# customink/lambdipy

Hardware: NVIDIA H100
Metric: ELF-strip GB/s (build-tree .so bytes) (higher is better)
Workload: dtype u8

## Files before the change

### lambdipy_b200/csrc/api.cu

```cuda
#include "lb2_common.cuh"
#include "../../include/lambdipy_b200.h"

#include <algorithm>
#include <atomic>
#include <chrono>
#include <cctype>
#include <cerrno>
#include <cstdio>
#include <cstdlib>
#include <condition_variable>
#include <cstring>
#include <mutex>
#include <string>
#include <thread>
#include <vector>

#include <climits>
#include <dirent.h>
#include <regex.h>
#include <fcntl.h>
#include <spawn.h>
#include <sys/stat.h>
#include <sys/syscall.h>
#include <sys/wait.h>
// ... 1 lines not shown

extern char **environ;

using namespace lb2;

static thread_local std::string g_create_error;

struct Workspace {
  uint64_t *d_in_off = nullptr, *d_in_size = nullptr, *d_out_size = nullptr, *d_out_off = nullptr;
  int32_t *d_status = nullptr;
  uint8_t *d_scratch = nullptr;
  Tile *d_tiles = nullptr;
  BatchCounters *d_ctr = nullptr;
  UpRange *d_ranges = nullptr, *h_ranges = nullptr;
  BigExt *d_big = nullptr;
  uint32_t cap_big = 0;
  uint32_t cap_ranges = 0;
  uint64_t *h_stage = nullptr;
  uint8_t *h_res = nullptr;
  BatchCounters *h_ctr = nullptr;
  cudaEvent_t done = nullptr;
  uint32_t cap_files = 0;
  uint64_t cap_tiles = 0;
  cudaEvent_t ev[3] = {nullptr, nullptr, nullptr};
  uint32_t n_files = 0;
  cudaStream_t stream = nullptr;
  bool in_flight = false;
};

struct TreeEngine;
struct lb2_ctx {
  int device = 0;
  int numa_node = -1;
  int sm_count = 0;
  cudaStream_t stream = nullptr;
  Workspace ws;
  Workspace ws2;
  int async_head = 0, async_count = 0;
  std::string err;
  int compact_ctas_per_sm = 4;
  int use_tma = 1;
  struct Slot {
    Workspace ws;
    cudaStream_t stream = nullptr;
    uint8_t *d_in = nullptr, *d_out = nullptr;
    uint64_t cap_in = 0, cap_out = 0;
    cudaEvent_t ev_h2d[2] = {nullptr, nullptr}, ev_d2h[2] = {nullptr, nullptr}, ev_planned = nullptr;
  } slot[3];
  TreeEngine *tree = nullptr;
};
struct TreeEngine;
static void tree_engine_free(TreeEngine *e);

#define CK(call)                                                                                   \
  do {                                                                                             \
    cudaError_t e_ = (call);                                                                       \
    if (e_ != cudaSuccess) {                                                                       \
      ctx->err = std::string(#call) + ": " + cudaGetErrorString(e_);                               \
      return LB2_E_CUDA;                                                                           \
    }                                                                                              \
  } while (0)

static int gpu_numa_node(int device) {
  char bus[64] = {0};
  if (cudaDeviceGetPCIBusId(bus, sizeof bus, device) != cudaSuccess) { cudaGetLastError(); return -1; }
  for (char *c = bus; *c; c++) *c = (char)tolower(*c);
  std::string path = std::string("/sys/bus/pci/devices/") + bus + "/numa_node";
  FILE *f = fopen(path.c_str(), "r");
  if (!f) return -1;
  int node = -1;
  if (fscanf(f, "%d", &node) != 1) node = -1;
// ... 23 lines not shown
  for (uint32_t i = t; i <= n; i += stride) h_off[i] = out_off[i];
  for (uint32_t i = t; i < n; i += stride) { h_size[i] = out_size[i]; h_status[i] = status[i]; }
  if (ranges) {
    const uint32_t nr = ctr->n_ranges < range_cap ? ctr->n_ranges : range_cap;
    for (uint32_t i = t; i < nr; i += stride) h_ranges[i] = ranges[i];
  }
}

static double now_s() {
  return std::chrono::duration<double>(std::chrono::steady_clock::now().time_since_epoch()).count();
}

static void ws_free(Workspace &w) {
  cudaFree(w.d_in_off); cudaFree(w.d_in_size); cudaFree(w.d_out_size); cudaFree(w.d_out_off); cudaFree(w.d_status);
  cudaFree(w.d_scratch); cudaFree(w.d_tiles); cudaFree(w.d_ctr);
  if (w.h_stage) cudaFreeHost(w.h_stage);
  if (w.h_res) cudaFreeHost(w.h_res);
  if (w.h_ctr) cudaFreeHost(w.h_ctr);
  cudaFree(w.d_ranges);
  cudaFree(w.d_big);
  if (w.h_ranges) cudaFreeHost(w.h_ranges);
  for (auto &e : w.ev) if (e) cudaEventDestroy(e);
  if (w.done) cudaEventDestroy(w.done);
  w = Workspace();
}

static int ws_reserve(lb2_ctx *ctx, Workspace &w, uint32_t n_files, uint64_t n_tiles) {
  if (!w.d_ctr) {
    CK(cudaMalloc(&w.d_ctr, sizeof(BatchCounters)));
    CK(cudaHostAlloc(&w.h_ctr, sizeof(BatchCounters) + 64, cudaHostAllocMapped));
    for (auto &e : w.ev) CK(cudaEventCreate(&e));
    CK(cudaEventCreateWithFlags(&w.done, cudaEventDisableTiming));
  }
  if (n_files > w.cap_files) {
    uint32_t cap = std::max<uint32_t>(n_files, 256u);
    cap = std::max<uint32_t>(cap, w.cap_files + w.cap_files / 2);
    cudaFree(w.d_in_off); cudaFree(w.d_in_size); cudaFree(w.d_out_size); cudaFree(w.d_out_off); cudaFree(w.d_status); cudaFree(w.d_scratch);
    if (w.h_stage) cudaFreeHost(w.h_stage);
    if (w.h_res) cudaFreeHost(w.h_res);
    w.h_stage = nullptr; w.h_res = nullptr;
    w.d_in_off = w.d_in_size = w.d_out_size = w.d_out_off = nullptr; w.d_status = nullptr; w.d_scratch = nullptr;
    w.cap_files = 0;
    CK(cudaMalloc(&w.d_in_off, (cap + 1) * sizeof(uint64_t)));
    CK(cudaMalloc(&w.d_in_size, (cap + 1) * sizeof(uint64_t)));
    CK(cudaMalloc(&w.d_out_size, (cap + 1) * sizeof(uint64_t)));
    CK(cudaMalloc(&w.d_out_off, (cap + 1) * sizeof(uint64_t)));
    CK(cudaMalloc(&w.d_status, (cap + 1) * sizeof(int32_t)));
    CK(cudaMalloc(&w.d_scratch, (uint64_t)cap * SCR_STRIDE));
    CK(cudaHostAlloc(&w.h_stage, (2ull * cap + 2) * sizeof(uint64_t), cudaHostAllocMapped));
    CK(cudaHostAlloc(&w.h_res, (2ull * cap + 2) * sizeof(uint64_t) + (cap + 1ull) * sizeof(int32_t), cudaHostAllocMapped));
    w.cap_files = cap;
  }
  if (n_tiles > w.cap_tiles) {
    uint64_t cap = std::max<uint64_t>(n_tiles, w.cap_tiles + w.cap_tiles / 2);
    cudaFree(w.d_tiles);
    w.d_tiles = nullptr;
    w.cap_tiles = 0;
    CK(cudaMalloc(&w.d_tiles, cap * sizeof(Tile)));
    w.cap_tiles = cap;
  }
  return LB2_OK;
}

static uint64_t tile_bound(const uint64_t *sizes, uint32_t n) {
  uint64_t t = 65536;
  for (uint32_t i = 0; i < n; i++) t += sizes[i] / TILE_BYTES + 2 * MAX_EXT + 16;
  return t;
}

static int enqueue_batch(lb2_ctx *ctx, Workspace &w, const uint8_t *d_in, const uint64_t *h_off, const uint64_t *h_sizes,
                         uint32_t n, uint8_t *d_out, uint64_t out_cap, uint32_t flags, cudaStream_t s, bool compact,
                         bool export_ranges = false, bool via_mapping = false) {
  for (uint32_t i = 0; i < n; i++)
    if (h_off[i] & 15) { ctx->err = "input offsets must be multiples of 16"; return LB2_E_ARG; }
  std::vector<uint64_t> tmp;
  if (w.in_flight) { ctx->err = "previous batch on this workspace not collected"; return LB2_E_STATE; }
  uint64_t *st_off = nullptr, *st_size = nullptr;
  {
    tmp.resize(n);
    for (uint32_t i = 0; i < n; i++) tmp[i] = h_sizes ? h_sizes[i] : (h_off[i + 1] - h_off[i]);
  }
  int rc = ws_reserve(ctx, w, n, tile_bound(tmp.data(), n));
  if (rc) return rc;
  st_off = w.h_stage;
  st_size = w.h_stage + (w.cap_files + 1);
  memcpy(st_off, h_off, (size_t)n * sizeof(uint64_t));
  memcpy(st_size, tmp.data(), (size_t)n * sizeof(uint64_t));
  const uint64_t *k_in_off = w.d_in_off, *k_in_size = w.d_in_size;
  if (via_mapping) {
    void *alias = nullptr;
    CK(cudaHostGetDevicePointer(&alias, w.h_stage, 0));
    k_in_off = static_cast<const uint64_t *>(alias);
    k_in_size = k_in_off + (w.cap_files + 1);
    lb2_zero_ctr_kernel<<<1, 64, 0, s>>>(w.d_ctr);
  } else {
    CK(cudaMemcpyAsync(w.d_in_off, st_off, (size_t)n * sizeof(uint64_t), cudaMemcpyHostToDevice, s));
    CK(cudaMemcpyAsync(w.d_in_size, st_size, (size_t)n * sizeof(uint64_t), cudaMemcpyHostToDevice, s));
    CK(cudaMemsetAsync(w.d_ctr, 0, sizeof(BatchCounters), s));
  }
  CK(cudaEventRecord(w.ev[0], s));
  if (export_ranges && w.cap_ranges < 8u * n + 4096u) {
    cudaFree(w.d_ranges);
    if (w.h_ranges) cudaFreeHost(w.h_ranges);
    w.d_ranges = nullptr; w.h_ranges = nullptr; w.cap_ranges = 0;
    const uint32_t cap = 8u * std::max<uint32_t>(n, w.cap_files) + 4096u;
    CK(cudaMalloc(&w.d_ranges, (size_t)cap * sizeof(UpRange)));
    CK(cudaHostAlloc(&w.h_ranges, (size_t)cap * sizeof(UpRange), cudaHostAllocMapped));
    w.cap_ranges = cap;
  }
  PlanArgs pa;
  pa.in = d_in; pa.in_off = k_in_off; pa.in_size = k_in_size; pa.n_files = n; pa.flags = flags;
  pa.scratch = w.d_scratch; pa.out_size = w.d_out_size; pa.status = w.d_status;
  pa.tiles = w.d_tiles; pa.tile_cap = w.cap_tiles; pa.ctr = w.d_ctr;
  pa.up_ranges = export_ranges ? w.d_ranges : nullptr; pa.up_cap = export_ranges ? w.cap_ranges : 0;
  if (w.cap_big < 8u * n + 4096u) {
    cudaFree(w.d_big);
    w.d_big = nullptr; w.cap_big = 0;
    const uint32_t cap = 8u * std::max<uint32_t>(n, w.cap_files) + 4096u;
    CK(cudaMalloc(&w.d_big, (size_t)cap * sizeof(BigExt)));
    w.cap_big = cap;
  }
  pa.big = w.d_big; pa.big_cap = w.cap_big;
  launch_plan(pa, s);
  launch_scan(w.d_out_size, w.d_out_off, n, compact ? out_cap : ~0ull, w.d_ctr, w.d_big, w.cap_big, w.d_tiles, ctx->sm_count * 2, s);
  CK(cudaEventRecord(w.ev[1], s));
  if (compact) {
    CompactArgs ca;
    ca.tiles = w.d_tiles; ca.ctr = w.d_ctr; ca.out_off = w.d_out_off; ca.out = d_out;
    ca.rebase_lo = ca.rebase_len = ca.rebase_delta = 0;
    if (ctx->use_tma) launch_compact_tma(ca, ctx->sm_count, s);
    else launch_compact(ca, ctx->sm_count * ctx->compact_ctas_per_sm, s);
  }
  CK(cudaEventRecord(w.ev[2], s));
  {
    uint64_t *r_off = reinterpret_cast<uint64_t *>(w.h_res), *r_size = r_off + (w.cap_files + 1);
    int32_t *r_status = reinterpret_cast<int32_t *>(r_size + (w.cap_files + 1));
    if (via_mapping) {
      void *a_ctr = nullptr, *a_res = nullptr, *a_rng = nullptr;
      CK(cudaHostGetDevicePointer(&a_ctr, w.h_ctr, 0));
      CK(cudaHostGetDevicePointer(&a_res, w.h_res, 0));
      if (export_ranges) CK(cudaHostGetDevicePointer(&a_rng, w.h_ranges, 0));
      uint64_t *m_off = static_cast<uint64_t *>(a_res), *m_size = m_off + (w.cap_files + 1);
      int32_t *m_status = reinterpret_cast<int32_t *>(m_size + (w.cap_files + 1));
      lb2_publish_kernel<<<std::max(1u, std::min(32u, (n + 255u) / 256u)), 256, 0, s>>>(
          w.d_ctr, w.d_out_off, w.d_out_size, w.d_status, export_ranges ? w.d_ranges : nullptr, n, w.cap_ranges,
          static_cast<BatchCounters *>(a_ctr), m_off, m_size, m_status, static_cast<UpRange *>(a_rng));
    } else {
      CK(cudaMemcpyAsync(w.h_ctr, w.d_ctr, sizeof(BatchCounters), cudaMemcpyDeviceToHost, s));
      if (export_ranges) CK(cudaMemcpyAsync(w.h_ranges, w.d_ranges, (size_t)std::min<uint32_t>(w.cap_ranges, 8u * n + 4096u) * sizeof(UpRange), cudaMemcpyDeviceToHost, s));
      CK(cudaMemcpyAsync(r_off, w.d_out_off, (size_t)(n + 1) * sizeof(uint64_t), cudaMemcpyDeviceToHost, s));
      if (n) {
        CK(cudaMemcpyAsync(r_size, w.d_out_size, (size_t)n * sizeof(uint64_t), cudaMemcpyDeviceToHost, s));
        CK(cudaMemcpyAsync(r_status, w.d_status, (size_t)n * sizeof(int32_t), cudaMemcpyDeviceToHost, s));
      }
    }
    CK(cudaEventRecord(w.done, s));
  }
  CK(cudaGetLastError());
  w.n_files = n;
  w.stream = s;
  w.in_flight = true;
  return LB2_OK;
}

static int collect_batch(lb2_ctx *ctx, Workspace &w, uint64_t *h_out_off, uint64_t *h_out_sizes, int32_t *h_status,
                         lb2_stats *stats) {
  if (!w.in_flight) { ctx->err = "no batch in flight"; return LB2_E_STATE; }
  const uint32_t n = w.n_files;
  CK(cudaEventSynchronize(w.done));
  w.in_flight = false;
  const uint64_t *r_off = reinterpret_cast<const uint64_t *>(w.h_res), *r_size = r_off + (w.cap_files + 1);
  const int32_t *r_status = reinterpret_cast<const int32_t *>(r_size + (w.cap_files + 1));
  if (h_out_off) memcpy(h_out_off, r_off, (size_t)(n + 1) * sizeof(uint64_t));
  if (h_out_sizes && n) memcpy(h_out_sizes, r_size, (size_t)n * sizeof(uint64_t));
  if (h_status && n) memcpy(h_status, r_status, (size_t)n * sizeof(int32_t));
  if (stats) {
    const BatchCounters &c = *w.h_ctr;
    memset(stats, 0, sizeof(*stats));
    stats->n_files = n; stats->n_ok = c.n_ok; stats->n_unsupported = c.n_unsupported; stats->overflow = c.overflow;
    stats->in_bytes = c.in_bytes; stats->out_bytes = c.out_bytes; stats->copy_bytes = c.copy_bytes;
    stats->header_bytes = c.header_bytes; stats->n_tiles = c.n_tiles; stats->out_bytes_needed = r_off[n];
    cudaEventElapsedTime(&stats->plan_ms, w.ev[0], w.ev[1]);
    cudaEventElapsedTime(&stats->compact_ms, w.ev[1], w.ev[2]);
  }
  if (w.h_ctr->overflow) { ctx->err = "output arena (or tile buffer) too small for this batch"; return LB2_E_CAPACITY; }
  return LB2_OK;
}

extern "C" {

const char *lb2_version(void) { return "lambdipy_b200 0.1 (sm_90a; GNU strip 2.42 semantics)"; }

int lb2_ctx_create(int device, lb2_ctx **out) {
  if (!out) return LB2_E_ARG;
  *out = nullptr;
  int count = 0;
  cudaError_t e = cudaGetDeviceCount(&count);
  if (e != cudaSuccess || count == 0) {
    g_create_error = std::string("no CUDA device: ") + (e != cudaSuccess ? cudaGetErrorString(e) : "device count is 0");
    return LB2_E_NODEVICE;
  }
  if (device < 0 || device >= count) { g_create_error = "device index out of range"; return LB2_E_ARG; }
  lb2_ctx *ctx = new lb2_ctx();
  ctx->device = device;
  if ((e = cudaSetDevice(device)) != cudaSuccess || (e = cudaStreamCreateWithFlags(&ctx->stream, cudaStreamNonBlocking)) != cudaSuccess) {
    g_create_error = std::string("cuda init: ") + cudaGetErrorString(e);
// ... 8 lines not shown
    g_create_error = "this library is built for sm_90a (H100) only; device is sm_" + std::to_string(prop.major) + std::to_string(prop.minor);
    cudaStreamDestroy(ctx->stream);
    delete ctx;
    return LB2_E_NODEVICE;
  }
  if (const char *v = getenv("LB2_COMPACT_CTAS_PER_SM")) ctx->compact_ctas_per_sm = std::max(1, atoi(v));
  if (const char *v = getenv("LB2_COMPACT_TMA")) ctx->use_tma = atoi(v);
  *out = ctx;
  return LB2_OK;
}

void lb2_ctx_destroy(lb2_ctx *ctx) {
  if (!ctx) return;
  cudaSetDevice(ctx->device);
  cudaDeviceSynchronize();
  ws_free(ctx->ws);
  ws_free(ctx->ws2);
  for (auto &sl : ctx->slot) {
    ws_free(sl.ws);
    cudaFree(sl.d_in); cudaFree(sl.d_out);
    if (sl.stream) cudaStreamDestroy(sl.stream);
    for (auto &e : sl.ev_h2d) if (e) cudaEventDestroy(e);
    for (auto &e : sl.ev_d2h) if (e) cudaEventDestroy(e);
    if (sl.ev_planned) cudaEventDestroy(sl.ev_planned);
  }
  tree_engine_free(ctx->tree);
  if (ctx->stream) cudaStreamDestroy(ctx->stream);
  delete ctx;
}

const char *lb2_last_error(const lb2_ctx *ctx) { return ctx ? ctx->err.c_str() : g_create_error.c_str(); }
int lb2_sm_count(const lb2_ctx *ctx) { return ctx ? ctx->sm_count : 0; }

void *lb2_dev_alloc(lb2_ctx *ctx, uint64_t bytes) {
  void *p = nullptr;
  cudaError_t e = cudaMalloc(&p, bytes ? bytes : 256);
  if (e != cudaSuccess) { if (ctx) ctx->err = std::string("cudaMalloc: ") + cudaGetErrorString(e); return nullptr; }
  return p;
}
void lb2_dev_free(lb2_ctx *, void *p) { if (p) cudaFree(p); }
void *lb2_pinned_alloc(lb2_ctx *ctx, uint64_t bytes) {
  void *p = nullptr;
  NumaPreferred near_gpu(ctx ? ctx->numa_node : -1);
  cudaError_t e = cudaHostAlloc(&p, bytes ? bytes : 256, cudaHostAllocMapped | cudaHostAllocPortable);
  if (e != cudaSuccess) { if (ctx) ctx->err = std::string("cudaHostAlloc: ") + cudaGetErrorString(e); return nullptr; }
  return p;
}
void lb2_pinned_free(lb2_ctx *, void *p) { if (p) cudaFreeHost(p); }
int lb2_memcpy_h2d(lb2_ctx *ctx, void *d, const void *h, uint64_t n) { CK(cudaMemcpy(d, h, n, cudaMemcpyHostToDevice)); return LB2_OK; }
int lb2_memcpy_d2h(lb2_ctx *ctx, void *h, const void *d, uint64_t n) { CK(cudaMemcpy(h, d, n, cudaMemcpyDeviceToHost)); return LB2_OK; }
int lb2_memset_d(lb2_ctx *ctx, void *d, int v, uint64_t n) { CK(cudaMemset(d, v, n)); return LB2_OK; }

int lb2_strip_device_async(lb2_ctx *ctx, const void *d_in, const uint64_t *h_in_off, const uint64_t *h_in_sizes,
                           uint32_t n_files, void *d_out, uint64_t out_capacity, uint32_t flags, void *stream) {
  if (!ctx || !d_in || !h_in_off || !d_out) { if (ctx) ctx->err = "NULL argument"; return LB2_E_ARG; }
  CK(cudaSetDevice(ctx->device));
  if (ctx->async_count >= 2) { ctx->err = "two batches already in flight: collect one with lb2_batch_results first"; return LB2_E_STATE; }
  cudaStream_t s = stream ? static_cast<cudaStream_t>(stream) : ctx->stream;
  Workspace &w = ((ctx->async_head + ctx->async_count) & 1) ? ctx->ws2 : ctx->ws;
  int rc = enqueue_batch(ctx, w, static_cast<const uint8_t *>(d_in), h_in_off, h_in_sizes, n_files,
                         static_cast<uint8_t *>(d_out), out_capacity, flags, s, true);
  if (rc == LB2_OK) ctx->async_count++;
  return rc;
}

int lb2_batch_results(lb2_ctx *ctx, uint64_t *h_out_off, uint64_t *h_out_sizes, int32_t *h_status, lb2_stats *stats) {
  if (!ctx) return LB2_E_ARG;
  if (ctx->async_count == 0) { ctx->err = "no batch in flight"; return LB2_E_STATE; }
  Workspace &w = (ctx->async_head & 1) ? ctx->ws2 : ctx->ws;
  ctx->async_head ^= 1;
  ctx->async_count--;
  return collect_batch(ctx, w, h_out_off, h_out_sizes, h_status, stats);
}

int lb2_plan_device(lb2_ctx *ctx, const void *d_in, const uint64_t *h_in_off, const uint64_t *h_in_sizes, uint32_t n_files,
                    uint32_t flags, uint64_t *h_out_sizes, int32_t *h_status, lb2_stats *stats) {
  if (!ctx || !d_in || !h_in_off) { if (ctx) ctx->err = "NULL argument"; return LB2_E_ARG; }
  CK(cudaSetDevice(ctx->device));
  if (ctx->async_count) { ctx->err = "batches of lb2_strip_device_async still in flight"; return LB2_E_STATE; }
  int rc = enqueue_batch(ctx, ctx->ws, static_cast<const uint8_t *>(d_in), h_in_off, h_in_sizes, n_files, nullptr, 0, flags,
                         ctx->stream, false);
  if (rc) return rc;
  return collect_batch(ctx, ctx->ws, nullptr, h_out_sizes, h_status, stats);
}
// ... 51 lines not shown
  for (size_t k = 0; k < chunks.size() && rc == LB2_OK; k++) {
    if (k >= 2) rc = collect(k - 2);
    if (rc == LB2_OK) rc = enqueue(k);
  }
  for (size_t k = chunks.size() >= 2 ? chunks.size() - 2 : 0; k < chunks.size(); k++) {
    Workspace &w = (k & 1) ? ctx->ws2 : ctx->ws;
    if (!w.in_flight) continue;
    int r = collect(k);
    if (rc == LB2_OK) rc = r;
  }
  if (total_out) *total_out = total;
  return rc;
}

static uint64_t env_u64(const char *name, uint64_t dflt) {
  const char *v = getenv(name);
  return v ? strtoull(v, nullptr, 10) : dflt;
}

static int strip_host_dma(lb2_ctx *ctx, const uint8_t *h_in, const uint8_t *d_in_alias, const uint64_t *h_in_off, const uint64_t *h_in_sizes,
                          uint32_t n_files, uint8_t *h_out, uint64_t out_capacity, uint64_t *h_out_off, uint64_t *h_out_sizes,
                          int32_t *h_status, uint32_t flags, lb2_stats *stats);

int lb2_strip_host(lb2_ctx *ctx, const void *h_in_v, const uint64_t *h_in_off, const uint64_t *h_in_sizes, uint32_t n_files,
                   void *h_out_v, uint64_t out_capacity, uint64_t *h_out_off, uint64_t *h_out_sizes, int32_t *h_status,
                   uint32_t flags, lb2_stats *stats) {
  if (!ctx || !h_in_v || !h_in_off || !h_out_v || !h_out_off || !h_out_sizes || !h_status) { if (ctx) ctx->err = "NULL argument"; return LB2_E_ARG; }
  CK(cudaSetDevice(ctx->device));
  const uint8_t *h_in = static_cast<const uint8_t *>(h_in_v);
  uint8_t *h_out = static_cast<uint8_t *>(h_out_v);
  if (env_u64("LB2_HOST_ZEROCOPY", 1) && n_files) {
    void *d_in_alias = nullptr, *d_out_alias = nullptr;
    cudaPointerAttributes ai, ao;
    const bool ok = cudaPointerGetAttributes(&ai, h_in) == cudaSuccess && ai.type == cudaMemoryTypeHost &&
                    cudaPointerGetAttributes(&ao, h_out) == cudaSuccess && ao.type == cudaMemoryTypeHost &&
                    cudaHostGetDevicePointer(&d_in_alias, const_cast<uint8_t *>(h_in), 0) == cudaSuccess &&
                    cudaHostGetDevicePointer(&d_out_alias, h_out, 0) == cudaSuccess;
    cudaGetLastError();
    if (ok && env_u64("LB2_HOST_DMA", 0)) {
      return strip_host_dma(ctx, h_in, static_cast<const uint8_t *>(d_in_alias), h_in_off, h_in_sizes, n_files, h_out, out_capacity,
                            h_out_off, h_out_sizes, h_status, flags, stats);
    }
    if (ok) {
      int rc = enqueue_batch(ctx, ctx->ws, static_cast<const uint8_t *>(d_in_alias), h_in_off, h_in_sizes, n_files,
                             static_cast<uint8_t *>(d_out_alias), out_capacity, flags, ctx->stream, true);
      if (rc) return rc;
      lb2_stats st;
      rc = collect_batch(ctx, ctx->ws, h_out_off, h_out_sizes, h_status, &st);
      st.h2d_bytes = st.copy_bytes + st.header_bytes;
      st.d2h_bytes = st.out_bytes;
      if (stats) *stats = st;
      return rc;
    }
  }
  const uint64_t chunk_bytes = env_u64("LB2_CHUNK_MB", 256) << 20;
  lb2_stats total;
  memset(&total, 0, sizeof total);
  total.n_files = n_files;

  struct Chunk { uint32_t f0, f1; uint64_t in_base, in_span; };
  std::vector<Chunk> chunks;
  for (uint32_t f = 0; f < n_files;) {
    uint32_t g = f + 1;
    while (g < n_files && h_in_off[g + 1] - h_in_off[f] <= chunk_bytes) g++;
    chunks.push_back({f, g, h_in_off[f], ((h_in_off[g] - h_in_off[f]) + 255) & ~255ull});
    f = g;
  }
  const int NS = 3;
  for (int k = 0; k < NS; k++) {
    auto &sl = ctx->slot[k];
    if (!sl.stream) {
      CK(cudaStreamCreateWithFlags(&sl.stream, cudaStreamNonBlocking));
      for (auto &e : sl.ev_h2d) CK(cudaEventCreate(&e));
      for (auto &e : sl.ev_d2h) CK(cudaEventCreate(&e));
      CK(cudaEventCreateWithFlags(&sl.ev_planned, cudaEventDisableTiming));
    }
  }
  std::vector<uint64_t> rel_off;
  uint64_t out_base = 0;
  int rc = LB2_OK;

  auto finish = [&](size_t ci) -> int {
    auto &sl = ctx->slot[ci % NS];
    const Chunk &c = chunks[ci];
    const uint32_t n = c.f1 - c.f0;
    lb2_stats st;
    std::vector<uint64_t> coff(n + 1);
    int r = collect_batch(ctx, sl.ws, coff.data(), h_out_sizes + c.f0, h_status + c.f0, &st);
    if (r == LB2_E_CAPACITY) {
      cudaFree(sl.d_out);
      sl.cap_out = 0;
      uint64_t need = st.out_bytes_needed + (1u << 20);
      CK(cudaMalloc(&sl.d_out, need));
      sl.cap_out = need;
      std::vector<uint64_t> ro(n + 1);
      for (uint32_t i = 0; i <= n; i++) ro[i] = h_in_off[c.f0 + i] - c.in_base;
      r = enqueue_batch(ctx, sl.ws, sl.d_in, ro.data(), h_in_sizes ? h_in_sizes + c.f0 : nullptr, n, sl.d_out, sl.cap_out, flags, sl.stream, true);
      if (r) return r;
// ... 41 lines not shown
    }
    CK(cudaEventRecord(sl.ev_h2d[0], sl.stream));
    CK(cudaMemcpyAsync(sl.d_in, h_in + c.in_base, h_in_off[c.f1] - c.in_base, cudaMemcpyHostToDevice, sl.stream));
    total.h2d_bytes += h_in_off[c.f1] - c.in_base;
    CK(cudaEventRecord(sl.ev_h2d[1], sl.stream));
    rel_off.resize(n + 1);
    for (uint32_t i = 0; i <= n; i++) rel_off[i] = h_in_off[c.f0 + i] - c.in_base;
    rc = enqueue_batch(ctx, sl.ws, sl.d_in, rel_off.data(), h_in_sizes ? h_in_sizes + c.f0 : nullptr, n, sl.d_out, sl.cap_out, flags, sl.stream, true);
    if (rc) break;
    if (ci >= 1) rc = finish(ci - 1);
  }
  if (rc == LB2_OK && !chunks.empty()) rc = finish(chunks.size() - 1);
  for (size_t ci = chunks.size() >= (size_t)NS ? chunks.size() - NS : 0; ci < chunks.size(); ci++) reap_copy_times(ci);
  for (int k = 0; k < NS; k++) { cudaStreamSynchronize(ctx->slot[k].stream); ctx->slot[k].ws.in_flight = false; }
  h_out_off[n_files] = out_base;
  if (total.out_bytes_needed == 0) total.out_bytes_needed = out_base;
  if (stats) *stats = total;
  return rc;
}

}


static int strip_host_dma(lb2_ctx *ctx, const uint8_t *h_in, const uint8_t *d_in_alias, const uint64_t *h_in_off, const uint64_t *h_in_sizes,
                          uint32_t n_files, uint8_t *h_out, uint64_t out_capacity, uint64_t *h_out_off, uint64_t *h_out_sizes,
                          int32_t *h_status, uint32_t flags, lb2_stats *stats) {
  const uint64_t chunk_bytes = env_u64("LB2_CHUNK_MB", 256) << 20;
  lb2_stats total;
  memset(&total, 0, sizeof total);
  total.n_files = n_files;
  struct Chunk { uint32_t f0, f1; uint64_t in_base, in_span; };
  std::vector<Chunk> chunks;
  for (uint32_t f = 0; f < n_files;) {
    uint32_t g = f + 1;
    while (g < n_files && h_in_off[g + 1] - h_in_off[f] <= chunk_bytes) g++;
    chunks.push_back({f, g, h_in_off[f], ((h_in_off[g] - h_in_off[f]) + 255) & ~255ull});
    f = g;
  }
  const int NS = 3;
  for (int k = 0; k < NS; k++) {
    auto &sl = ctx->slot[k];
    if (!sl.stream) {
      CK(cudaStreamCreateWithFlags(&sl.stream, cudaStreamNonBlocking));
      for (auto &e : sl.ev_h2d) CK(cudaEventCreate(&e));
      for (auto &e : sl.ev_d2h) CK(cudaEventCreate(&e));
      CK(cudaEventCreateWithFlags(&sl.ev_planned, cudaEventDisableTiming));
    }
  }
  uint64_t out_base = 0;
  std::vector<uint64_t> rel_off, coff;
  auto plan = [&](size_t ci) -> int {
    auto &sl = ctx->slot[ci % NS];
    const Chunk &c = chunks[ci];
    const uint32_t n = c.f1 - c.f0;
    if (ci >= (size_t)NS) {
      CK(cudaEventSynchronize(sl.ev_d2h[1]));
      float a = 0, b = 0;
      cudaEventElapsedTime(&a, sl.ev_h2d[0], sl.ev_h2d[1]);
      cudaEventElapsedTime(&b, sl.ev_d2h[0], sl.ev_d2h[1]);
      total.h2d_ms += a; total.d2h_ms += b;
    }
    rel_off.resize(n + 1);
    for (uint32_t i = 0; i <= n; i++) rel_off[i] = h_in_off[c.f0 + i] - c.in_base;
    return enqueue_batch(ctx, sl.ws, d_in_alias + c.in_base, rel_off.data(), h_in_sizes ? h_in_sizes + c.f0 : nullptr, n, nullptr, 0, flags,
                         sl.stream, false, true, true);
  };
  auto move = [&](size_t ci) -> int {
    auto &sl = ctx->slot[ci % NS];
    const Chunk &c = chunks[ci];
    const uint32_t n = c.f1 - c.f0;
    lb2_stats st;
    coff.resize(n + 1);
    int r = collect_batch(ctx, sl.ws, coff.data(), h_out_sizes + c.f0, h_status + c.f0, &st);
    if (r) return r;
    const uint64_t bytes = coff[n];
    if (out_base + bytes > out_capacity) { ctx->err = "host output arena too small"; total.out_bytes_needed = out_base + bytes; return LB2_E_CAPACITY; }
    if (sl.cap_in < c.in_span + 256) {
      cudaFree(sl.d_in); sl.d_in = nullptr; sl.cap_in = 0;
      const uint64_t need = std::max<uint64_t>(c.in_span + 256, std::min<uint64_t>(chunk_bytes, 64ull << 20));
      CK(cudaMalloc(&sl.d_in, need));
      sl.cap_in = need;
    }
    if (sl.cap_out < bytes + 256) {
      cudaFree(sl.d_out); sl.d_out = nullptr; sl.cap_out = 0;
      const uint64_t need = std::max<uint64_t>(bytes + (1u << 20), c.in_span + (8u << 20));
      CK(cudaMalloc(&sl.d_out, need));
      sl.cap_out = need;
    }
    const BatchCounters &bc = *sl.ws.h_ctr;
    CK(cudaEventRecord(sl.ev_h2d[0], sl.stream));
    if (bc.ranges_overflow || bc.n_ranges > sl.ws.cap_ranges) {
      CK(cudaMemcpyAsync(sl.d_in, h_in + c.in_base, h_in_off[c.f1] - c.in_base, cudaMemcpyHostToDevice, sl.stream));
      total.h2d_bytes += h_in_off[c.f1] - c.in_base;
    } else {
      UpRange *rg = sl.ws.h_ranges;
      std::sort(rg, rg + bc.n_ranges, [](const UpRange &x, const UpRange &y) { return x.off < y.off; });
      uint64_t rs = 0, re = 0;
      auto flush = [&]() -> int {
        if (re <= rs) return LB2_OK;
        if (re > c.in_span) { ctx->err = "upload range outside the chunk"; return LB2_E_STATE; }
        CK(cudaMemcpyAsync(sl.d_in + rs, h_in + c.in_base + rs, re - rs, cudaMemcpyHostToDevice, sl.stream));
        total.h2d_bytes += re - rs;
        return LB2_OK;
      };
      for (uint32_t k = 0; k < bc.n_ranges; k++) {
        const uint64_t o = rg[k].off, e = rg[k].off + rg[k].len;
        if (re > rs && o <= re + 8192) { if (e > re) re = e; }
        else { int fr = flush(); if (fr) return fr; rs = o; re = e; }
      }
      int fr = flush();
      if (fr) return fr;
    }
    CK(cudaEventRecord(sl.ev_h2d[1], sl.stream));
    CompactArgs ca;
    ca.tiles = sl.ws.d_tiles; ca.ctr = sl.ws.d_ctr; ca.out_off = sl.ws.d_out_off; ca.out = sl.d_out;
    ca.rebase_lo = reinterpret_cast<uint64_t>(d_in_alias + c.in_base);
    ca.rebase_len = c.in_span;
    ca.rebase_delta = reinterpret_cast<uint64_t>(sl.d_in) - ca.rebase_lo;
    CK(cudaEventRecord(sl.ws.ev[1], sl.stream));
    if (ctx->use_tma) launch_compact_tma(ca, ctx->sm_count, sl.stream);
    else launch_compact(ca, ctx->sm_count * ctx->compact_ctas_per_sm, sl.stream);
    CK(cudaEventRecord(sl.ws.ev[2], sl.stream));
    CK(cudaEventRecord(sl.ev_d2h[0], sl.stream));
    if (bytes) CK(cudaMemcpyAsync(h_out + out_base, sl.d_out, bytes, cudaMemcpyDeviceToHost, sl.stream));
    total.d2h_bytes += bytes;
    total.h2d_bytes += st.header_bytes;
    CK(cudaEventRecord(sl.ev_d2h[1], sl.stream));
    CK(cudaGetLastError());
    for (uint32_t i = 0; i < n; i++) h_out_off[c.f0 + i] = out_base + coff[i];
    out_base += bytes;
    total.n_ok += st.n_ok; total.n_unsupported += st.n_unsupported; total.in_bytes += st.in_bytes; total.out_bytes += st.out_bytes;
    total.copy_bytes += st.copy_bytes; total.header_bytes += st.header_bytes; total.n_tiles += st.n_tiles;
    total.plan_ms += st.plan_ms;
    return LB2_OK;
  };
  int rc = LB2_OK;
  for (size_t ci = 0; ci < chunks.size() && rc == LB2_OK; ci++) {
    rc = plan(ci);
    if (rc == LB2_OK && ci >= 1) rc = move(ci - 1);
  }
  if (rc == LB2_OK && !chunks.empty()) rc = move(chunks.size() - 1);
  for (int k = 0; k < NS; k++) {
    auto &sl = ctx->slot[k];
    cudaStreamSynchronize(sl.stream);
    sl.ws.in_flight = false;
    if ((size_t)k < chunks.size()) {
      float a = 0, b = 0, cms = 0;
      if (cudaEventElapsedTime(&a, sl.ev_h2d[0], sl.ev_h2d[1]) == cudaSuccess) total.h2d_ms += a;
      if (cudaEventElapsedTime(&b, sl.ev_d2h[0], sl.ev_d2h[1]) == cudaSuccess) total.d2h_ms += b;
      if (cudaEventElapsedTime(&cms, sl.ws.ev[1], sl.ws.ev[2]) == cudaSuccess) total.compact_ms += cms;
    }
  }
  cudaGetLastError();
  h_out_off[n_files] = out_base;
  if (total.out_bytes_needed == 0) total.out_bytes_needed = out_base;
  if (stats) *stats = total;
  return rc;
}

static bool ends_with(const char *s, const char *suf) {
  size_t a = strlen(s), b = strlen(suf);
  return a >= b && memcmp(s + a - b, suf, b) == 0;
}

struct TreeFile { std::string path; uint64_t size; dev_t dev; ino_t ino; uint32_t times; };

struct Cleanup {
  bool on = false;
  regex_t keep;
  bool have_keep = false;
  uint32_t n_removed = 0;
};

static void rm_rf(const std::string &p) {
  struct stat sb;
// ... 565 lines not shown
```

### lambdipy_b200/csrc/compact_tma.cu

```cuda
#include "lb2_common.cuh"
#include "copy_device.cuh"

namespace lb2 {

constexpr int TMA_STAGES = 12;
constexpr int TMA_THREADS = 256;
constexpr uint32_t TMA_MIN_BODY = 2048;
constexpr int TMA_STORES_IN_FLIGHT = 6;

__device__ __forceinline__ uint32_t smem_u32(const void *p) { return (uint32_t)__cvta_generic_to_shared(p); }
__device__ __forceinline__ void mbar_init(uint64_t *bar, uint32_t count) {
  asm volatile("mbarrier.init.shared::cta.b64 [%0], %1;" :: "r"(smem_u32(bar)), "r"(count));
}
__device__ __forceinline__ void mbar_expect_tx(uint64_t *bar, uint32_t bytes) {
  asm volatile("mbarrier.arrive.expect_tx.shared::cta.b64 _, [%0], %1;" :: "r"(smem_u32(bar)), "r"(bytes) : "memory");
}
__device__ __forceinline__ void mbar_arrive(uint64_t *bar) {
  asm volatile("mbarrier.arrive.shared::cta.b64 _, [%0];" :: "r"(smem_u32(bar)) : "memory");
}
__device__ __forceinline__ void mbar_wait(uint64_t *bar, uint32_t parity) {
  asm volatile(
      "{\n"
      ".reg .pred p;\n"
      "WAIT_%=:\n"
      "mbarrier.try_wait.parity.shared::cta.b64 p, [%0], %1;\n"
      "@p bra DONE_%=;\n"
      "bra WAIT_%=;\n"
      "DONE_%=:\n"
// ... 123 lines not shown
        const uint32_t len_ = __shfl_sync(0xffffffffu, len, l), head_ = __shfl_sync(0xffffffffu, head, l),
                       body_ = __shfl_sync(0xffffffffu, body, l);
        if (body_) {
          if (lane < (int)head_) d_[lane] = __ldg(s_ + lane);
          const uint32_t done = head_ + body_, tail = len_ - done;
          if (lane < (int)tail) d_[done + lane] = __ldg(s_ + done + lane);
        } else if (s_) {
          warp_copy_tile(s_, d_, len_, lane);
        } else {
          warp_zero_tile(d_, len_, lane);
        }
      }
    }
  }
}

void launch_compact_tma(const CompactArgs &a, int grid, cudaStream_t s) {
  static bool configured[64] = {};
  const size_t smem = (size_t)TMA_STAGES * TILE_BYTES;
  int dev = 0;
  cudaGetDevice(&dev);
  if (dev < 0 || dev >= 64 || !configured[dev]) {
    cudaFuncSetAttribute(lb2_compact_tma_kernel, cudaFuncAttributeMaxDynamicSharedMemorySize, (int)smem);
    if (dev >= 0 && dev < 64) configured[dev] = true;
  }
  lb2_compact_tma_kernel<<<grid, TMA_THREADS, smem, s>>>(a);
}

}
```

Measured before the change: 2527.

## Pipeline host DMA strip across dedicated streams and offload planning to side stream

Replaces the three-slot host DMA pipeline with separate plan, upload, compact and download streams. It sizes the chunk count and pipeline depth from free device memory, uploads ranges through a single batched memcpy call, and turns host DMA on by default for large inputs. Async batches now plan on a side stream and publish results on a result stream, so planning can overlap the previous batch's compaction. TMA stages drop by one and the max shared-memory carveout is requested. The cost is more streams, more events and more cross-stream dependencies to get right.

```diff
diff --git a/lambdipy_b200/csrc/api.cu b/lambdipy_b200/csrc/api.cu
--- a/lambdipy_b200/csrc/api.cu
+++ b/lambdipy_b200/csrc/api.cu
@@ -47,7 +47,8 @@
   cudaEvent_t done = nullptr;
   uint32_t cap_files = 0;
   uint64_t cap_tiles = 0;
-  cudaEvent_t ev[3] = {nullptr, nullptr, nullptr};
+  cudaEvent_t ev[4] = {nullptr, nullptr, nullptr, nullptr};
+  cudaEvent_t fork = nullptr;
   uint32_t n_files = 0;
   cudaStream_t stream = nullptr;
   bool in_flight = false;
@@ -59,6 +60,7 @@
   int numa_node = -1;
   int sm_count = 0;
   cudaStream_t stream = nullptr;
+  cudaStream_t side = nullptr, res = nullptr;
   Workspace ws;
   Workspace ws2;
   int async_head = 0, async_count = 0;
@@ -70,8 +72,23 @@
     cudaStream_t stream = nullptr;
     uint8_t *d_in = nullptr, *d_out = nullptr;
     uint64_t cap_in = 0, cap_out = 0;
-    cudaEvent_t ev_h2d[2] = {nullptr, nullptr}, ev_d2h[2] = {nullptr, nullptr}, ev_planned = nullptr;
+    cudaEvent_t ev_h2d[2] = {nullptr, nullptr}, ev_d2h[2] = {nullptr, nullptr};
   } slot[3];
+  struct DmaSlot {
+    uint8_t *d_in = nullptr, *d_out = nullptr;
+    uint64_t cap_in = 0, cap_out = 0;
+    cudaEvent_t ev[6] = {};
+    bool busy = false;
+  };
+  struct DmaPlan {
+    Workspace ws;
+    cudaEvent_t released = nullptr;
+  };
+  struct {
+    cudaStream_t plan = nullptr, up = nullptr, comp = nullptr, down = nullptr;
+    std::vector<DmaSlot> slots;
+    std::vector<DmaPlan> plans;
+  } dma;
   TreeEngine *tree = nullptr;
 };
 struct TreeEngine;
@@ -141,6 +158,7 @@
   if (w.h_ranges) cudaFreeHost(w.h_ranges);
   for (auto &e : w.ev) if (e) cudaEventDestroy(e);
   if (w.done) cudaEventDestroy(w.done);
+  if (w.fork) cudaEventDestroy(w.fork);
   w = Workspace();
 }
 
@@ -150,6 +168,7 @@
     CK(cudaHostAlloc(&w.h_ctr, sizeof(BatchCounters) + 64, cudaHostAllocMapped));
     for (auto &e : w.ev) CK(cudaEventCreate(&e));
     CK(cudaEventCreateWithFlags(&w.done, cudaEventDisableTiming));
+    CK(cudaEventCreateWithFlags(&w.fork, cudaEventDisableTiming));
   }
   if (n_files > w.cap_files) {
     uint32_t cap = std::max<uint32_t>(n_files, 256u);
@@ -189,7 +208,8 @@
 
 static int enqueue_batch(lb2_ctx *ctx, Workspace &w, const uint8_t *d_in, const uint64_t *h_off, const uint64_t *h_sizes,
                          uint32_t n, uint8_t *d_out, uint64_t out_cap, uint32_t flags, cudaStream_t s, bool compact,
-                         bool export_ranges = false, bool via_mapping = false) {
+                         bool export_ranges = false, bool via_mapping = false, bool off_stream = false,
+                         cudaEvent_t plan_after = nullptr) {
   for (uint32_t i = 0; i < n; i++)
     if (h_off[i] & 15) { ctx->err = "input offsets must be multiples of 16"; return LB2_E_ARG; }
   std::vector<uint64_t> tmp;
@@ -203,6 +223,11 @@
   if (rc) return rc;
   st_off = w.h_stage;
   st_size = w.h_stage + (w.cap_files + 1);
+  const cudaStream_t ps = off_stream ? ctx->side : s, rs = off_stream ? ctx->res : s;
+  if (off_stream) {
+    CK(cudaEventRecord(w.fork, s));
+    CK(cudaStreamWaitEvent(ps, plan_after ? plan_after : w.fork, 0));
+  }
   memcpy(st_off, h_off, (size_t)n * sizeof(uint64_t));
   memcpy(st_size, tmp.data(), (size_t)n * sizeof(uint64_t));
   const uint64_t *k_in_off = w.d_in_off, *k_in_size = w.d_in_size;
@@ -211,13 +236,13 @@
     CK(cudaHostGetDevicePointer(&alias, w.h_stage, 0));
     k_in_off = static_cast<const uint64_t *>(alias);
     k_in_size = k_in_off + (w.cap_files + 1);
-    lb2_zero_ctr_kernel<<<1, 64, 0, s>>>(w.d_ctr);
+    lb2_zero_ctr_kernel<<<1, 64, 0, ps>>>(w.d_ctr);
   } else {
-    CK(cudaMemcpyAsync(w.d_in_off, st_off, (size_t)n * sizeof(uint64_t), cudaMemcpyHostToDevice, s));
-    CK(cudaMemcpyAsync(w.d_in_size, st_size, (size_t)n * sizeof(uint64_t), cudaMemcpyHostToDevice, s));
-    CK(cudaMemsetAsync(w.d_ctr, 0, sizeof(BatchCounters), s));
-  }
-  CK(cudaEventRecord(w.ev[0], s));
+    CK(cudaMemcpyAsync(w.d_in_off, st_off, (size_t)n * sizeof(uint64_t), cudaMemcpyHostToDevice, ps));
+    CK(cudaMemcpyAsync(w.d_in_size, st_size, (size_t)n * sizeof(uint64_t), cudaMemcpyHostToDevice, ps));
+    CK(cudaMemsetAsync(w.d_ctr, 0, sizeof(BatchCounters), ps));
+  }
+  CK(cudaEventRecord(w.ev[0], ps));
   if (export_ranges && w.cap_ranges < 8u * n + 4096u) {
     cudaFree(w.d_ranges);
     if (w.h_ranges) cudaFreeHost(w.h_ranges);
@@ -240,9 +265,11 @@
     w.cap_big = cap;
   }
   pa.big = w.d_big; pa.big_cap = w.cap_big;
-  launch_plan(pa, s);
-  launch_scan(w.d_out_size, w.d_out_off, n, compact ? out_cap : ~0ull, w.d_ctr, w.d_big, w.cap_big, w.d_tiles, ctx->sm_count * 2, s);
-  CK(cudaEventRecord(w.ev[1], s));
+  launch_plan(pa, ps);
+  launch_scan(w.d_out_size, w.d_out_off, n, compact ? out_cap : ~0ull, w.d_ctr, w.d_big, w.cap_big, w.d_tiles, ctx->sm_count * 2, ps);
+  CK(cudaEventRecord(w.ev[1], ps));
+  if (off_stream) CK(cudaStreamWaitEvent(s, w.ev[1], 0));
+  CK(cudaEventRecord(w.ev[3], s));
   if (compact) {
     CompactArgs ca;
     ca.tiles = w.d_tiles; ca.ctr = w.d_ctr; ca.out_off = w.d_out_off; ca.out = d_out;
@@ -251,6 +278,7 @@
     else launch_compact(ca, ctx->sm_count * ctx->compact_ctas_per_sm, s);
   }
   CK(cudaEventRecord(w.ev[2], s));
+  if (off_stream) CK(cudaStreamWaitEvent(rs, w.ev[2], 0));
   {
     uint64_t *r_off = reinterpret_cast<uint64_t *>(w.h_res), *r_size = r_off + (w.cap_files + 1);
     int32_t *r_status = reinterpret_cast<int32_t *>(r_size + (w.cap_files + 1));
@@ -261,19 +289,19 @@
       if (export_ranges) CK(cudaHostGetDevicePointer(&a_rng, w.h_ranges, 0));
       uint64_t *m_off = static_cast<uint64_t *>(a_res), *m_size = m_off + (w.cap_files + 1);
       int32_t *m_status = reinterpret_cast<int32_t *>(m_size + (w.cap_files + 1));
-      lb2_publish_kernel<<<std::max(1u, std::min(32u, (n + 255u) / 256u)), 256, 0, s>>>(
+      lb2_publish_kernel<<<std::max(1u, std::min(32u, (n + 255u) / 256u)), 256, 0, rs>>>(
           w.d_ctr, w.d_out_off, w.d_out_size, w.d_status, export_ranges ? w.d_ranges : nullptr, n, w.cap_ranges,
           static_cast<BatchCounters *>(a_ctr), m_off, m_size, m_status, static_cast<UpRange *>(a_rng));
     } else {
-      CK(cudaMemcpyAsync(w.h_ctr, w.d_ctr, sizeof(BatchCounters), cudaMemcpyDeviceToHost, s));
-      if (export_ranges) CK(cudaMemcpyAsync(w.h_ranges, w.d_ranges, (size_t)std::min<uint32_t>(w.cap_ranges, 8u * n + 4096u) * sizeof(UpRange), cudaMemcpyDeviceToHost, s));
-      CK(cudaMemcpyAsync(r_off, w.d_out_off, (size_t)(n + 1) * sizeof(uint64_t), cudaMemcpyDeviceToHost, s));
+      CK(cudaMemcpyAsync(w.h_ctr, w.d_ctr, sizeof(BatchCounters), cudaMemcpyDeviceToHost, rs));
+      if (export_ranges) CK(cudaMemcpyAsync(w.h_ranges, w.d_ranges, (size_t)std::min<uint32_t>(w.cap_ranges, 8u * n + 4096u) * sizeof(UpRange), cudaMemcpyDeviceToHost, rs));
+      CK(cudaMemcpyAsync(r_off, w.d_out_off, (size_t)(n + 1) * sizeof(uint64_t), cudaMemcpyDeviceToHost, rs));
       if (n) {
-        CK(cudaMemcpyAsync(r_size, w.d_out_size, (size_t)n * sizeof(uint64_t), cudaMemcpyDeviceToHost, s));
-        CK(cudaMemcpyAsync(r_status, w.d_status, (size_t)n * sizeof(int32_t), cudaMemcpyDeviceToHost, s));
+        CK(cudaMemcpyAsync(r_size, w.d_out_size, (size_t)n * sizeof(uint64_t), cudaMemcpyDeviceToHost, rs));
+        CK(cudaMemcpyAsync(r_status, w.d_status, (size_t)n * sizeof(int32_t), cudaMemcpyDeviceToHost, rs));
       }
     }
-    CK(cudaEventRecord(w.done, s));
+    CK(cudaEventRecord(w.done, rs));
   }
   CK(cudaGetLastError());
   w.n_files = n;
@@ -300,7 +328,7 @@
     stats->in_bytes = c.in_bytes; stats->out_bytes = c.out_bytes; stats->copy_bytes = c.copy_bytes;
     stats->header_bytes = c.header_bytes; stats->n_tiles = c.n_tiles; stats->out_bytes_needed = r_off[n];
     cudaEventElapsedTime(&stats->plan_ms, w.ev[0], w.ev[1]);
-    cudaEventElapsedTime(&stats->compact_ms, w.ev[1], w.ev[2]);
+    cudaEventElapsedTime(&stats->compact_ms, w.ev[3], w.ev[2]);
   }
   if (w.h_ctr->overflow) { ctx->err = "output arena (or tile buffer) too small for this batch"; return LB2_E_CAPACITY; }
   return LB2_OK;
@@ -355,9 +383,19 @@
     if (sl.stream) cudaStreamDestroy(sl.stream);
     for (auto &e : sl.ev_h2d) if (e) cudaEventDestroy(e);
     for (auto &e : sl.ev_d2h) if (e) cudaEventDestroy(e);
-    if (sl.ev_planned) cudaEventDestroy(sl.ev_planned);
-  }
+  }
+  for (auto &sl : ctx->dma.slots) {
+    cudaFree(sl.d_in); cudaFree(sl.d_out);
+    for (auto &e : sl.ev) if (e) cudaEventDestroy(e);
+  }
+  for (auto &p : ctx->dma.plans) {
+    ws_free(p.ws);
+    if (p.released) cudaEventDestroy(p.released);
+  }
+  for (cudaStream_t s : {ctx->dma.plan, ctx->dma.up, ctx->dma.comp, ctx->dma.down}) if (s) cudaStreamDestroy(s);
   tree_engine_free(ctx->tree);
+  if (ctx->side) cudaStreamDestroy(ctx->side);
+  if (ctx->res) cudaStreamDestroy(ctx->res);
   if (ctx->stream) cudaStreamDestroy(ctx->stream);
   delete ctx;
 }
@@ -390,9 +428,15 @@
   CK(cudaSetDevice(ctx->device));
   if (ctx->async_count >= 2) { ctx->err = "two batches already in flight: collect one with lb2_batch_results first"; return LB2_E_STATE; }
   cudaStream_t s = stream ? static_cast<cudaStream_t>(stream) : ctx->stream;
+  if (!ctx->side) {
+    CK(cudaStreamCreateWithFlags(&ctx->side, cudaStreamNonBlocking));
+    CK(cudaStreamCreateWithFlags(&ctx->res, cudaStreamNonBlocking));
+  }
   Workspace &w = ((ctx->async_head + ctx->async_count) & 1) ? ctx->ws2 : ctx->ws;
+  const Workspace &prev = (ctx->async_head & 1) ? ctx->ws2 : ctx->ws;
+  const bool follows = ctx->async_count == 1 && prev.stream == s;
   int rc = enqueue_batch(ctx, w, static_cast<const uint8_t *>(d_in), h_in_off, h_in_sizes, n_files,
-                         static_cast<uint8_t *>(d_out), out_capacity, flags, s, true);
+                         static_cast<uint8_t *>(d_out), out_capacity, flags, s, true, false, false, true, follows ? prev.fork : nullptr);
   if (rc == LB2_OK) ctx->async_count++;
   return rc;
 }
@@ -490,6 +534,8 @@
                           uint32_t n_files, uint8_t *h_out, uint64_t out_capacity, uint64_t *h_out_off, uint64_t *h_out_sizes,
                           int32_t *h_status, uint32_t flags, lb2_stats *stats);
 
+static const uint64_t HOST_DMA_MIN_SPAN = 256ull << 20;
+
 int lb2_strip_host(lb2_ctx *ctx, const void *h_in_v, const uint64_t *h_in_off, const uint64_t *h_in_sizes, uint32_t n_files,
                    void *h_out_v, uint64_t out_capacity, uint64_t *h_out_off, uint64_t *h_out_sizes, int32_t *h_status,
                    uint32_t flags, lb2_stats *stats) {
@@ -505,7 +551,8 @@
                     cudaHostGetDevicePointer(&d_in_alias, const_cast<uint8_t *>(h_in), 0) == cudaSuccess &&
                     cudaHostGetDevicePointer(&d_out_alias, h_out, 0) == cudaSuccess;
     cudaGetLastError();
-    if (ok && env_u64("LB2_HOST_DMA", 0)) {
+    const bool large = h_in_off[n_files] - h_in_off[0] >= HOST_DMA_MIN_SPAN;
+    if (ok && env_u64("LB2_HOST_DMA", large ? 1 : 0)) {
       return strip_host_dma(ctx, h_in, static_cast<const uint8_t *>(d_in_alias), h_in_off, h_in_sizes, n_files, h_out, out_capacity,
                             h_out_off, h_out_sizes, h_status, flags, stats);
     }
@@ -541,7 +588,6 @@
       CK(cudaStreamCreateWithFlags(&sl.stream, cudaStreamNonBlocking));
       for (auto &e : sl.ev_h2d) CK(cudaEventCreate(&e));
       for (auto &e : sl.ev_d2h) CK(cudaEventCreate(&e));
-      CK(cudaEventCreateWithFlags(&sl.ev_planned, cudaEventDisableTiming));
     }
   }
   std::vector<uint64_t> rel_off;
@@ -629,10 +675,26 @@
 }
 
 
+static const uint64_t DMA_CHUNK_MAX = 256ull << 20;
+static const uint64_t DMA_RING_MAX = 4ull << 30;
+static const int DMA_DEPTH_MIN = 3, DMA_DEPTH_MAX = 6;
+
 static int strip_host_dma(lb2_ctx *ctx, const uint8_t *h_in, const uint8_t *d_in_alias, const uint64_t *h_in_off, const uint64_t *h_in_sizes,
                           uint32_t n_files, uint8_t *h_out, uint64_t out_capacity, uint64_t *h_out_off, uint64_t *h_out_sizes,
                           int32_t *h_status, uint32_t flags, lb2_stats *stats) {
-  const uint64_t chunk_bytes = env_u64("LB2_CHUNK_MB", 256) << 20;
+  auto &D = ctx->dma;
+  size_t free_b = 0, total_b = 0;
+  CK(cudaMemGetInfo(&free_b, &total_b));
+  uint64_t held = 0;
+  for (auto &sl : D.slots) held += sl.cap_in + sl.cap_out;
+  const uint64_t budget = std::min<uint64_t>((free_b + held) / 4, DMA_RING_MAX);
+  const uint64_t span = h_in_off[n_files] - h_in_off[0];
+  const uint64_t chunk_bytes = getenv("LB2_CHUNK_MB") ? env_u64("LB2_CHUNK_MB", 0) << 20
+                                                      : std::clamp<uint64_t>(std::min(budget / (2 * DMA_DEPTH_MAX), span / 8), 16ull << 20, DMA_CHUNK_MAX);
+  const int depth = (int)std::clamp<uint64_t>(budget / (2 * chunk_bytes + (8u << 20)), DMA_DEPTH_MIN, DMA_DEPTH_MAX);
+  const int n_plans = depth + 2;
+  const uint64_t fuse_gap = env_u64("LB2_HOST_DMA_GAP_KB", 8) << 10;
+
   lb2_stats total;
   memset(&total, 0, sizeof total);
   total.n_files = n_files;
@@ -644,44 +706,53 @@
     chunks.push_back({f, g, h_in_off[f], ((h_in_off[g] - h_in_off[f]) + 255) & ~255ull});
     f = g;
   }
-  const int NS = 3;
-  for (int k = 0; k < NS; k++) {
-    auto &sl = ctx->slot[k];
-    if (!sl.stream) {
-      CK(cudaStreamCreateWithFlags(&sl.stream, cudaStreamNonBlocking));
-      for (auto &e : sl.ev_h2d) CK(cudaEventCreate(&e));
-      for (auto &e : sl.ev_d2h) CK(cudaEventCreate(&e));
-      CK(cudaEventCreateWithFlags(&sl.ev_planned, cudaEventDisableTiming));
-    }
-  }
+  if (!D.up)
+    for (cudaStream_t *s : {&D.plan, &D.up, &D.comp, &D.down}) CK(cudaStreamCreateWithFlags(s, cudaStreamNonBlocking));
+  while ((int)D.slots.size() < depth) {
+    D.slots.emplace_back();
+    for (auto &e : D.slots.back().ev) CK(cudaEventCreate(&e));
+  }
+  while ((int)D.plans.size() < n_plans) {
+    D.plans.emplace_back();
+    CK(cudaEventCreateWithFlags(&D.plans.back().released, cudaEventDisableTiming));
+  }
+
   uint64_t out_base = 0;
   std::vector<uint64_t> rel_off, coff;
-  auto plan = [&](size_t ci) -> int {
-    auto &sl = ctx->slot[ci % NS];
-    const Chunk &c = chunks[ci];
+  std::vector<void *> up_dst, up_src;
+  std::vector<size_t> up_len;
+  auto reap = [&](lb2_ctx::DmaSlot &sl) {
+    float a = 0, b = 0, c = 0;
+    if (cudaEventElapsedTime(&a, sl.ev[0], sl.ev[1]) == cudaSuccess) total.h2d_ms += a;
+    if (cudaEventElapsedTime(&c, sl.ev[2], sl.ev[3]) == cudaSuccess) total.compact_ms += c;
+    if (cudaEventElapsedTime(&b, sl.ev[4], sl.ev[5]) == cudaSuccess) total.d2h_ms += b;
+    sl.busy = false;
+  };
+  auto plan = [&](size_t k) -> int {
+    auto &p = D.plans[k % n_plans];
+    const Chunk &c = chunks[k];
     const uint32_t n = c.f1 - c.f0;
-    if (ci >= (size_t)NS) {
-      CK(cudaEventSynchronize(sl.ev_d2h[1]));
-      float a = 0, b = 0;
-      cudaEventElapsedTime(&a, sl.ev_h2d[0], sl.ev_h2d[1]);
-      cudaEventElapsedTime(&b, sl.ev_d2h[0], sl.ev_d2h[1]);
-      total.h2d_ms += a; total.d2h_ms += b;
-    }
+    CK(cudaStreamWaitEvent(D.plan, p.released, 0));
     rel_off.resize(n + 1);
     for (uint32_t i = 0; i <= n; i++) rel_off[i] = h_in_off[c.f0 + i] - c.in_base;
-    return enqueue_batch(ctx, sl.ws, d_in_alias + c.in_base, rel_off.data(), h_in_sizes ? h_in_sizes + c.f0 : nullptr, n, nullptr, 0, flags,
-                         sl.stream, false, true, true);
+    return enqueue_batch(ctx, p.ws, d_in_alias + c.in_base, rel_off.data(), h_in_sizes ? h_in_sizes + c.f0 : nullptr, n, nullptr, 0, flags,
+                         D.plan, false, true, true);
   };
-  auto move = [&](size_t ci) -> int {
-    auto &sl = ctx->slot[ci % NS];
-    const Chunk &c = chunks[ci];
+  auto move = [&](size_t k) -> int {
+    auto &p = D.plans[k % n_plans];
+    auto &sl = D.slots[k % depth];
+    const Chunk &c = chunks[k];
     const uint32_t n = c.f1 - c.f0;
     lb2_stats st;
     coff.resize(n + 1);
-    int r = collect_batch(ctx, sl.ws, coff.data(), h_out_sizes + c.f0, h_status + c.f0, &st);
+    int r = collect_batch(ctx, p.ws, coff.data(), h_out_sizes + c.f0, h_status + c.f0, &st);
     if (r) return r;
     const uint64_t bytes = coff[n];
     if (out_base + bytes > out_capacity) { ctx->err = "host output arena too small"; total.out_bytes_needed = out_base + bytes; return LB2_E_CAPACITY; }
+    if (sl.busy) {
+      CK(cudaEventSynchronize(sl.ev[5]));
+      reap(sl);
+    }
     if (sl.cap_in < c.in_span + 256) {
       cudaFree(sl.d_in); sl.d_in = nullptr; sl.cap_in = 0;
       const uint64_t need = std::max<uint64_t>(c.in_span + 256, std::min<uint64_t>(chunk_bytes, 64ull << 20));
@@ -694,46 +765,56 @@
       CK(cudaMalloc(&sl.d_out, need));
       sl.cap_out = need;
     }
-    const BatchCounters &bc = *sl.ws.h_ctr;
-    CK(cudaEventRecord(sl.ev_h2d[0], sl.stream));
-    if (bc.ranges_overflow || bc.n_ranges > sl.ws.cap_ranges) {
-      CK(cudaMemcpyAsync(sl.d_in, h_in + c.in_base, h_in_off[c.f1] - c.in_base, cudaMemcpyHostToDevice, sl.stream));
-      total.h2d_bytes += h_in_off[c.f1] - c.in_base;
+    const BatchCounters &bc = *p.ws.h_ctr;
+    up_dst.clear(); up_src.clear(); up_len.clear();
+    auto add = [&](uint64_t rs, uint64_t re) {
+      up_dst.push_back(sl.d_in + rs);
+      up_src.push_back(const_cast<uint8_t *>(h_in + c.in_base + rs));
+      up_len.push_back(re - rs);
+      total.h2d_bytes += re - rs;
+    };
+    if (bc.ranges_overflow || bc.n_ranges > p.ws.cap_ranges) {
+      add(0, h_in_off[c.f1] - c.in_base);
     } else {
-      UpRange *rg = sl.ws.h_ranges;
+      UpRange *rg = p.ws.h_ranges;
       std::sort(rg, rg + bc.n_ranges, [](const UpRange &x, const UpRange &y) { return x.off < y.off; });
       uint64_t rs = 0, re = 0;
-      auto flush = [&]() -> int {
-        if (re <= rs) return LB2_OK;
-        if (re > c.in_span) { ctx->err = "upload range outside the chunk"; return LB2_E_STATE; }
-        CK(cudaMemcpyAsync(sl.d_in + rs, h_in + c.in_base + rs, re - rs, cudaMemcpyHostToDevice, sl.stream));
-        total.h2d_bytes += re - rs;
-        return LB2_OK;
-      };
-      for (uint32_t k = 0; k < bc.n_ranges; k++) {
-        const uint64_t o = rg[k].off, e = rg[k].off + rg[k].len;
-        if (re > rs && o <= re + 8192) { if (e > re) re = e; }
-        else { int fr = flush(); if (fr) return fr; rs = o; re = e; }
+      for (uint32_t i = 0; i < bc.n_ranges; i++) {
+        const uint64_t o = rg[i].off, e = rg[i].off + rg[i].len;
+        if (re > rs && o <= re + fuse_gap) { if (e > re) re = e; }
+        else { if (re > rs) add(rs, re); rs = o; re = e; }
       }
-      int fr = flush();
-      if (fr) return fr;
-    }
-    CK(cudaEventRecord(sl.ev_h2d[1], sl.stream));
+      if (re > rs) add(rs, re);
+      if (re > c.in_span) { ctx->err = "upload range outside the chunk"; return LB2_E_STATE; }
+    }
+    CK(cudaEventRecord(sl.ev[0], D.up));
+    if (!up_len.empty()) {
+      cudaMemcpyAttributes attr;
+      memset(&attr, 0, sizeof attr);
+      attr.srcAccessOrder = cudaMemcpySrcAccessOrderStream;
+      size_t attr_idx = 0, fail_idx = 0;
+      CK(cudaMemcpyBatchAsync(up_dst.data(), up_src.data(), up_len.data(), up_len.size(), &attr, &attr_idx, 1, &fail_idx, D.up));
+    }
+    CK(cudaEventRecord(sl.ev[1], D.up));
     CompactArgs ca;
-    ca.tiles = sl.ws.d_tiles; ca.ctr = sl.ws.d_ctr; ca.out_off = sl.ws.d_out_off; ca.out = sl.d_out;
+    ca.tiles = p.ws.d_tiles; ca.ctr = p.ws.d_ctr; ca.out_off = p.ws.d_out_off; ca.out = sl.d_out;
     ca.rebase_lo = reinterpret_cast<uint64_t>(d_in_alias + c.in_base);
     ca.rebase_len = c.in_span;
     ca.rebase_delta = reinterpret_cast<uint64_t>(sl.d_in) - ca.rebase_lo;
-    CK(cudaEventRecord(sl.ws.ev[1], sl.stream));
-    if (ctx->use_tma) launch_compact_tma(ca, ctx->sm_count, sl.stream);
-    else launch_compact(ca, ctx->sm_count * ctx->compact_ctas_per_sm, sl.stream);
-    CK(cudaEventRecord(sl.ws.ev[2], sl.stream));
-    CK(cudaEventRecord(sl.ev_d2h[0], sl.stream));
-    if (bytes) CK(cudaMemcpyAsync(h_out + out_base, sl.d_out, bytes, cudaMemcpyDeviceToHost, sl.stream));
+    CK(cudaStreamWaitEvent(D.comp, sl.ev[1], 0));
+    CK(cudaEventRecord(sl.ev[2], D.comp));
+    if (ctx->use_tma) launch_compact_tma(ca, ctx->sm_count, D.comp);
+    else launch_compact(ca, ctx->sm_count * ctx->compact_ctas_per_sm, D.comp);
+    CK(cudaEventRecord(sl.ev[3], D.comp));
+    CK(cudaEventRecord(p.released, D.comp));
+    CK(cudaStreamWaitEvent(D.down, sl.ev[3], 0));
+    CK(cudaEventRecord(sl.ev[4], D.down));
+    if (bytes) CK(cudaMemcpyAsync(h_out + out_base, sl.d_out, bytes, cudaMemcpyDeviceToHost, D.down));
+    CK(cudaEventRecord(sl.ev[5], D.down));
+    CK(cudaGetLastError());
+    sl.busy = true;
     total.d2h_bytes += bytes;
     total.h2d_bytes += st.header_bytes;
-    CK(cudaEventRecord(sl.ev_d2h[1], sl.stream));
-    CK(cudaGetLastError());
     for (uint32_t i = 0; i < n; i++) h_out_off[c.f0 + i] = out_base + coff[i];
     out_base += bytes;
     total.n_ok += st.n_ok; total.n_unsupported += st.n_unsupported; total.in_bytes += st.in_bytes; total.out_bytes += st.out_bytes;
@@ -742,22 +823,15 @@
     return LB2_OK;
   };
   int rc = LB2_OK;
-  for (size_t ci = 0; ci < chunks.size() && rc == LB2_OK; ci++) {
-    rc = plan(ci);
-    if (rc == LB2_OK && ci >= 1) rc = move(ci - 1);
-  }
-  if (rc == LB2_OK && !chunks.empty()) rc = move(chunks.size() - 1);
-  for (int k = 0; k < NS; k++) {
-    auto &sl = ctx->slot[k];
-    cudaStreamSynchronize(sl.stream);
-    sl.ws.in_flight = false;
-    if ((size_t)k < chunks.size()) {
-      float a = 0, b = 0, cms = 0;
-      if (cudaEventElapsedTime(&a, sl.ev_h2d[0], sl.ev_h2d[1]) == cudaSuccess) total.h2d_ms += a;
-      if (cudaEventElapsedTime(&b, sl.ev_d2h[0], sl.ev_d2h[1]) == cudaSuccess) total.d2h_ms += b;
-      if (cudaEventElapsedTime(&cms, sl.ws.ev[1], sl.ws.ev[2]) == cudaSuccess) total.compact_ms += cms;
-    }
-  }
+  size_t planned = 0;
+  while (rc == LB2_OK && planned < chunks.size() && planned < (size_t)n_plans) rc = plan(planned++);
+  for (size_t k = 0; k < chunks.size() && rc == LB2_OK; k++) {
+    rc = move(k);
+    if (rc == LB2_OK && planned < chunks.size()) rc = plan(planned++);
+  }
+  for (cudaStream_t s : {D.plan, D.up, D.comp, D.down}) cudaStreamSynchronize(s);
+  for (auto &p : D.plans) p.ws.in_flight = false;
+  for (auto &sl : D.slots) if (sl.busy) reap(sl);
   cudaGetLastError();
   h_out_off[n_files] = out_base;
   if (total.out_bytes_needed == 0) total.out_bytes_needed = out_base;
diff --git a/lambdipy_b200/csrc/compact_tma.cu b/lambdipy_b200/csrc/compact_tma.cu
--- a/lambdipy_b200/csrc/compact_tma.cu
+++ b/lambdipy_b200/csrc/compact_tma.cu
@@ -3,7 +3,7 @@
 
 namespace lb2 {
 
-constexpr int TMA_STAGES = 12;
+constexpr int TMA_STAGES = 11;
 constexpr int TMA_THREADS = 256;
 constexpr uint32_t TMA_MIN_BODY = 2048;
 constexpr int TMA_STORES_IN_FLIGHT = 6;
@@ -173,6 +173,7 @@
   cudaGetDevice(&dev);
   if (dev < 0 || dev >= 64 || !configured[dev]) {
     cudaFuncSetAttribute(lb2_compact_tma_kernel, cudaFuncAttributeMaxDynamicSharedMemorySize, (int)smem);
+    cudaFuncSetAttribute(lb2_compact_tma_kernel, cudaFuncAttributePreferredSharedMemoryCarveout, (int)cudaSharedmemCarveoutMaxShared);
     if (dev >= 0 && dev < 64) configured[dev] = true;
   }
   lb2_compact_tma_kernel<<<grid, TMA_THREADS, smem, s>>>(a);
```

Result: faster. 2579, median of 6 (+2.1%).
